# naturerobots/mesh_navigation

Measured on NVIDIA H100. Metric: vertex-relaxations/sec, higher is better.
Workload: dtype f64 update / f32 store

## Files before the change

mesh_navigation_b200/csrc/band_engine.cuh:

```cuda
#pragma once
#include <cooperative_groups.h>
#include <cstdint>

#include "wavefront_math.cuh"

namespace mnb {
namespace cg = cooperative_groups;

constexpr uint32_t INF_BITS = 0x7f800000u;
constexpr int STAGNATION_ROUNDS = 24;

constexpr uint32_t EXT_POOL = 0x80000000u;
struct EvTime { float a1, a2, a3; uint32_t root, ext, self; };
__device__ __forceinline__ EvTime ev_normal(float key, uint32_t id) { EvTime t; t.a1 = key; t.a2 = 0.0f; t.a3 = 0.0f; t.root = id; t.ext = 0u; t.self = id; return t; }
struct Label { float d; EvTime t; };
__device__ __forceinline__ uint4 state_inf() { return make_uint4(INF_BITS, INF_BITS, 0u, 0u); }

struct TimeAlg {
  const uint32_t* pool = nullptr;
  __device__ __forceinline__ uint32_t id2_of(const EvTime& t) const {
    return t.a3 == 0.0f ? t.self : ((t.ext & EXT_POOL) ? __ldcg(&pool[(t.ext & ~EXT_POOL) + 1]) : t.ext);
  }
  __device__ __forceinline__ uint32_t id3_of(const EvTime& t) const {
    return (t.ext & EXT_POOL) ? __ldcg(&pool[(t.ext & ~EXT_POOL) + 2]) : t.self;
  }
  __device__ __forceinline__ uint32_t levels_of(const EvTime& t) const {
    return t.a2 == 0.0f ? 1u : (t.a3 == 0.0f ? 2u : ((t.ext & EXT_POOL) ? __ldcg(&pool[t.ext & ~EXT_POOL]) : 3u));
  }
  __device__ __noinline__ bool less_tail(const EvTime x, const EvTime y) const {
    const uint32_t i2x = id2_of(x), i2y = id2_of(y);
    if (i2x != i2y) return i2x < i2y;
    if (x.a3 != y.a3) return x.a3 < y.a3;
    if (x.a3 == 0.0f) return false;
    const uint32_t i3x = id3_of(x), i3y = id3_of(y);
    if (i3x != i3y) return i3x < i3y;
    const uint32_t nx = levels_of(x), ny = levels_of(y);
    const uint32_t ox = x.ext & ~EXT_POOL, oy = y.ext & ~EXT_POOL;
    for (uint32_t i = 4;; ++i) {
      if (i > nx) return i <= ny;
      if (i > ny) return false;
      const uint32_t kx = __ldcg(&pool[ox + 3 + 2 * (i - 4)]), ky = __ldcg(&pool[oy + 3 + 2 * (i - 4)]);
      if (kx != ky) return kx < ky;
      const uint32_t ix = __ldcg(&pool[ox + 4 + 2 * (i - 4)]), iy = __ldcg(&pool[oy + 4 + 2 * (i - 4)]);
      if (ix != iy) return ix < iy;
    }
// ... 180 lines not shown
};

template <int CS>
__device__ __forceinline__ void group_sync(unsigned int* bar = nullptr) {
  if constexpr (CS == 1) {
    __syncthreads();
  } else if constexpr (CS == 0) {
    (void)bar;
    cg::this_grid().sync();
  } else {
    cg::this_cluster().sync();
  }
}

template <int CAP_>
struct StageT {
  static constexpr int CAP = CAP_;
  static constexpr int SW_CAP = 1024;
  uint32_t buf[CAP];
  unsigned int n;
  unsigned int base;
  unsigned int m_tau;
  unsigned int lo;
};
using Stage = StageT<3072>;
struct SweepStage {
  uint32_t seen[Stage::SW_CAP];
  uint4 lab[Stage::SW_CAP];
  uint16_t dl[Stage::SW_CAP];
  unsigned int dn[2];
};
constexpr uint32_t SEEN_NEVER = 0xffffffffu;

__device__ __forceinline__ unsigned int stage_push(Stage& st, uint32_t v, uint32_t* list_next, unsigned int* count_next) {
  const unsigned int p = atomicAdd(&st.n, 1u);
  if (p < Stage::CAP) st.buf[p] = v;
  else list_next[atomicAdd(count_next, 1u)] = v;
  return p;
}
__device__ __forceinline__ void stage_push_seen(Stage& st, SweepStage& ss, uint32_t v, uint32_t seen, const uint4& label_bits,
                                                uint32_t* list_next, unsigned int* count_next) {
  const unsigned int p = stage_push(st, v, list_next, count_next);
  if (p < Stage::SW_CAP) { ss.seen[p] = seen; ss.lab[p] = label_bits; }
}

template <class S>
__device__ __forceinline__ void stage_flush(S& st, uint32_t* list_next, unsigned int* count_next,
                                            unsigned int* g_m_tau, unsigned int* g_lo) {
  __syncthreads();
  const unsigned int n = st.n < (unsigned)S::CAP ? st.n : (unsigned)S::CAP;
  if (threadIdx.x == 0) {
    st.base = n ? atomicAdd(count_next, n) : 0u;
    if (st.m_tau != INF_BITS) atomicMin(g_m_tau, st.m_tau);
    if (st.lo != INF_BITS) atomicMin(g_lo, st.lo);
  }
  __syncthreads();
  const unsigned int base = st.base;
  for (unsigned int i = threadIdx.x; i < n; i += blockDim.x) list_next[base + i] = st.buf[i];
  __syncthreads();
  if (threadIdx.x == 0) { st.n = 0; st.m_tau = INF_BITS; st.lo = INF_BITS; }
}

template <int CS, class P>
__device__ void run_band_rounds(P& prob, GroupCtl* ctl, uint32_t* list0, uint32_t* list1, uint32_t* mark,
                                Stage& st, const float delta, const uint32_t gthreads, const uint32_t gtid,
                                const int has_robot, const uint32_t r0, const uint32_t r1, const uint32_t r2,
                                const double goal_dist_offset, const volatile int* cancel_flag,
                                const float band_end_init, const uint32_t max_rounds) {
  float band_end_prev = band_end_init;
  unsigned long long my_recomputes = 0, my_settled = 0, my_skipped = 0;
  float lo_best = -1.0f; int stagnant = 0;
  prob.strict = 0;
  uint32_t r = 0;
  for (;; ++r) {
    const uint32_t slot = r % 3, prev = (r + 2) % 3, next = (r + 1) % 3;
    const unsigned int n = __ldcg(&ctl->count[slot]);
// ... 124 lines not shown
    {
      my_mtau = fminf(my_mtau, prob.deferred_m);
      prob.deferred_m = __uint_as_float(INF_BITS);
      const unsigned int wm = __reduce_min_sync(0xffffffffu, __float_as_uint(my_mtau));
      const unsigned int wl = __reduce_min_sync(0xffffffffu, __float_as_uint(my_lo));
      if ((threadIdx.x & 31) == 0) {
        if (wm != INF_BITS) atomicMin(&st.m_tau, wm);
        if (wl != INF_BITS) atomicMin(&st.lo, wl);
      }
    }
    stage_flush(st, list_n, &ctl->count[next], &ctl->m_tau[slot], &ctl->lo[slot]);
    band_end_prev = band_end;
    group_sync<CS>(ctl->barrier);
  }
  atomicAdd(&ctl->recomputes, my_recomputes);
  atomicAdd(&ctl->settled, my_settled);
  if (my_skipped) atomicAdd(&ctl->skipped, my_skipped);
  if (gtid == 0) {
    ctl->rounds += r;
    if (prob.strict) ctl->strict_armed += 1;
    if (r > max_rounds) ctl->watchdog = 1;
    ctl->goal_bits = min(ctl->goal_ring[0], ctl->goal_ring[1]);
  }
}

template <int CS, bool SW, class P>
__device__ void run_band_rounds_sub8(P& prob, GroupCtl* ctl, uint32_t* list0, uint32_t* list1, uint32_t* mark,
                                     Stage& st, const float delta, const uint32_t gthreads, const uint32_t gtid,
                                     const int has_robot, const uint32_t r0, const uint32_t r1, const uint32_t r2,
                                     const double goal_dist_offset, const volatile int* cancel_flag,
                                     const float band_end_init, const uint32_t max_rounds, const int n_sweeps_arg,
                                     SweepStage* ss, const uint32_t n_vertices) {
  const int n_sweeps = SW ? n_sweeps_arg : 0;
  bool rescanned = false;
  float band_end_prev = band_end_init;
  unsigned long long my_recomputes = 0, my_settled = 0, my_skipped = 0;
  float lo_best = -1.0f; int stagnant = 0;
  prob.strict = 0;
  const uint32_t j = threadIdx.x & 7;
  const uint32_t nblk = gthreads / blockDim.x, blk = gtid / blockDim.x;
  uint32_t r = 0;
  for (;; ++r) {
    const uint32_t slot = r % 3, prev = (r + 2) % 3, next = (r + 1) % 3;
    const unsigned int n = __ldcg(&ctl->count[slot]);
    const float m_prev = __uint_as_float(__ldcg(&ctl->m_tau[prev]));
    const float lo_prev = __uint_as_float(__ldcg(&ctl->lo[prev]));
    const unsigned int goal_b = __ldcg(&ctl->goal_ring[r & 1]);
    const float goal = __uint_as_float(goal_b);
    if constexpr (P::HAS_GOAL_TIME) if (has_robot && goal_b != INF_BITS) {
      prob.goal_t.a1 = __uint_as_float(__ldcg(&ctl->goal_time[0])); prob.goal_t.root = __ldcg(&ctl->goal_time[1]);
      prob.goal_t.a2 = __uint_as_float(__ldcg(&ctl->goal_time[2])); prob.goal_t.a3 = __uint_as_float(__ldcg(&ctl->goal_time[3]));
      prob.goal_t.ext = __ldcg(&ctl->goal_time[4]); prob.goal_t.self = __ldcg(&ctl->goal_time[5]);
    }
    const unsigned int stop = __ldcg(&ctl->stop_ring[r & 1]);
    const bool need_rescan = has_robot && goal_b != INF_BITS && !rescanned;
    if (stop || r > max_rounds) break;
    if (!need_rescan && n == 0) break;
    if (!need_rescan && r > 0 && __float_as_uint(m_prev) == INF_BITS &&
        (__float_as_uint(lo_prev) == INF_BITS || lo_prev > goal)) break;
    if (r > 0 && __float_as_uint(m_prev) != INF_BITS && !(lo_prev > lo_best)) { if (++stagnant >= STAGNATION_ROUNDS) prob.strict = 1; }
    else { stagnant = 0; if (lo_prev > lo_best) lo_best = lo_prev; }
#ifdef MNB_EMU_ACTIVE
    if (gtid == 0 && getenv("MNB_EMU_TRACE")) fprintf(stderr, "[round %u] list %u m_prev %g lo_prev %g strict %d\n", r, n, m_prev, lo_prev, prob.strict);
#endif
    float delta_r = delta;
    if constexpr (SW) {
// ... 56 lines not shown
          my_mtau = fminf(my_mtau, fminf(tau, nt.a1));
        }
        my_lo = fminf(my_lo, nt.a1);
        if constexpr (SW) {
          if (fresh) stage_push_seen(st, *ss, c, v0, prob.pack_label(c, nd, nt), list_n, &ctl->count[next]);
          else if (changed) ss->lab[slot] = prob.pack_label(c, nd, nt);
        } else {
          stage_push(st, c, list_n, &ctl->count[next]);
        }
      }
      if constexpr (SW) if (n_sweeps > 0) {
        __syncwarp();
        if (changed) {
          if (ix.x != -1 && deg <= 8) { atomicAdd(&prob.ver[ix.x], 1u); if constexpr (P::TWO_SOURCES) atomicAdd(&prob.ver[ix.y], 1u); }
          if (j == 0 && deg > 8) prob.activate(c, [&](uint32_t x) { atomicAdd(&prob.ver[x], 1u); });
        }
      }
      if (has && __float_as_uint(nd) != INF_BITS && mk == MARK_CAND) {
        if (ix.x != -1) {
          if (!prob.prefetch_marks) { mk1 = __ldcg(&mark[ix.x]); if (P::TWO_SOURCES) mk2 = __ldcg(&mark[ix.y]); }
          if (mk1 == MARK_NONE && prob.eligible((uint32_t)ix.x) && atomicCAS(&mark[ix.x], MARK_NONE, MARK_CAND) == MARK_NONE)
            { if constexpr (SW) stage_push_seen(st, *ss, (uint32_t)ix.x, SEEN_NEVER, state_inf(), list_n, &ctl->count[next]); else stage_push(st, (uint32_t)ix.x, list_n, &ctl->count[next]); }
          if (P::TWO_SOURCES && mk2 == MARK_NONE && prob.eligible((uint32_t)ix.y) && atomicCAS(&mark[ix.y], MARK_NONE, MARK_CAND) == MARK_NONE)
            { if constexpr (SW) stage_push_seen(st, *ss, (uint32_t)ix.y, SEEN_NEVER, state_inf(), list_n, &ctl->count[next]); else stage_push(st, (uint32_t)ix.y, list_n, &ctl->count[next]); }
        }
        if (j == 0 && deg > 8)
          prob.activate(c, [&](uint32_t x) {
            if (__ldcg(&mark[x]) == MARK_NONE && prob.eligible(x) && atomicCAS(&mark[x], MARK_NONE, MARK_CAND) == MARK_NONE)
              { if constexpr (SW) stage_push_seen(st, *ss, x, SEEN_NEVER, state_inf(), list_n, &ctl->count[next]); else stage_push(st, x, list_n, &ctl->count[next]); }
          });
        if (j == 0) mark[c] = MARK_CAND_ACT;
      }
    };
    const unsigned int cnt = n > blk ? (n - blk + nblk - 1) / nblk : 0u;
    for (unsigned int qb = (threadIdx.x >> 5) * 4u; qb < cnt; qb += (blockDim.x >> 3)) {
      const unsigned int q = qb + ((threadIdx.x & 31) >> 3);
      bool has = q < cnt;
      uint32_t c = 0;
      if (has) c = __ldcg(&list_r[(size_t)q * nblk + blk]);
      Label old = prob.load_label(has ? c : 0u);
      int4 ix = prob.load_row_idx(has ? c : 0u, j);
      float4 w = prob.load_row_w(has ? c : 0u, j);
      const uint32_t mk = __ldcg(&mark[has ? c : 0u]);
      uint32_t v0 = 0;
      if constexpr (SW) if (n_sweeps > 0) v0 = __ldcg(&prob.ver[has ? c : 0u]);
      const float d = old.d, tau = old.t.a1;
      if (has && tau < m_prev && tau < band_end_prev && tau < settle_cap) {
        if (j == 0) {
          mark[c] = MARK_FIXED;
          my_settled++;
          if (has_robot && (c == r0 || c == r1 || c == r2)) {
            if (atomicSub(&ctl->robot_left, 1) == 1) {
              float bd = d; EvTime bt = old.t;
              const uint32_t rv[3] = {r0, r1, r2};
              for (int k = 0; k < 3; ++k) {
                const Label so = prob.load_label(rv[k]);
                if (prob.tless(bt, so.t)) { bt = so.t; bd = so.d; }
              }
              ctl->goal_time[0] = __float_as_uint(bt.a1); ctl->goal_time[1] = bt.root; ctl->goal_time[2] = __float_as_uint(bt.a2);
            ctl->goal_time[3] = __float_as_uint(bt.a3); ctl->goal_time[4] = bt.ext; ctl->goal_time[5] = bt.self;
            atomicMin(&ctl->goal_ring[(r + 1) & 1], __float_as_uint((float)((double)bd + goal_dist_offset)));
            }
          }
        }
        has = false;
      }
      if constexpr (P::CAN_SKIP) if (skip_ok && has) {
        const uint32_t le = __ldcg(&prob.last_eval[c]), dr = __ldcg(&prob.dirty_round[c]);
        const float em = __uint_as_float(__ldcg(&prob.excl_min[c]));
        if (le != 0u && dr < le && !(band_end > em)) {
          if (j == 0) {
            my_lo = fminf(my_lo, tau);
            my_skipped++;
            if constexpr (SW) stage_push_seen(st, *ss, c, v0, prob.pack_label(c, old.d, old.t), list_n, &ctl->count[next]);
            else stage_push(st, c, list_n, &ctl->count[next]);
          }
          has = false;
        }
      }
      evaluate(has, c, old, ix, w, mk, v0, true, 0u);
    }
#ifdef MNB_GRID_TIMING
    const long long tps = clock64();
#endif
#ifdef MNB_GRID_TIMING
    if (gtid == 0) { ctl->t_ph[0] += (unsigned long long)(tps - tp0); ctl->t_ph[2] += cnt; }
#endif
    if constexpr (SW) for (int sw = 0; sw < n_sweeps; ++sw) {
#ifdef MNB_GRID_TIMING
      const long long tq0 = clock64();
#endif
      __syncthreads();
      const unsigned int ns = min(st.n, (unsigned int)Stage::SW_CAP);
      unsigned int* dcur = &ss->dn[sw & 1];
      if (threadIdx.x == 0) ss->dn[(sw + 1) & 1] = 0;
      for (unsigned int i = threadIdx.x; i < ns; i += blockDim.x) {
        const uint32_t c = st.buf[i];
        const uint32_t v0 = __ldcg(&prob.ver[c]);
        if (v0 != ss->seen[i]) { ss->seen[i] = v0; ss->dl[atomicAdd(dcur, 1u)] = (uint16_t)i; }
      }
      __syncthreads();
      const unsigned int dn = *dcur;
#ifdef MNB_GRID_TIMING
      const long long tq1 = clock64();
#endif
#ifdef MNB_GRID_TIMING
      if (gtid == 0) { ctl->t_ph[3] += dn; ctl->t_ph[4] += ns; ctl->t_ph[5] += (unsigned long long)(tq1 - tq0); }
#endif
      for (unsigned int ib = (threadIdx.x >> 5) * 4u; ib < dn; ib += (blockDim.x >> 3)) {
        const unsigned int i = ib + ((threadIdx.x & 31) >> 3);
        const bool has = i < dn;
        const uint32_t slot = has ? ss->dl[i] : 0u;
        const uint32_t c = has ? st.buf[slot] : 0u;
        const Label old = has ? prob.unpack_label(c, ss->lab[slot]) : prob.unpack_label(0u, state_inf());
// ... 46 lines not shown
```

mesh_navigation_b200/csrc/batch_engine.cuh:

```cuda
#pragma once
#include "problems.cuh"

namespace mnb {

struct BatchSeeds { uint32_t s0, s1, s2, noexpand; float seed_max; };
constexpr uint32_t LIST_ACTIVATED = 0x80000000u;

struct BatchGroup {
  uint4* state; uint32_t* root_arr; uint32_t* ext_arr; uint32_t* chg; uint32_t* mark; uint32_t* pool; uint32_t pool_cap; GroupCtl* ctl;
  uint4* skipw;
};

template <class Args>
__device__ __forceinline__ void batch_make_problem(const Args& a, const BatchGroup& G, const BatchSeeds& sd, int strict,
                                                   CvpEllProblemT<false>& prob) {
  prob.cor_ptr = a.cor_ptr; prob.cor_idx = a.cor_idx; prob.cor_w = a.cor_w; prob.cost = a.cost; prob.invalid = a.invalid;
  prob.ell_idx = a.ell_idx; prob.ell_w = a.ell_w; prob.ell_geo = a.ell_geo;
  prob.state = G.state; prob.ext_arr = G.ext_arr; prob.root_arr = G.root_arr; prob.chg = G.chg;
  prob.pool_w = G.pool; prob.pool = G.pool; prob.pool_cap = G.pool_cap; prob.pool_top = &G.ctl->pool_top; prob.pool_overflow = &G.ctl->pool_overflow;
  prob.ver = nullptr; prob.deferred_m = __uint_as_float(INF_BITS); prob.pred = nullptr; prob.dir = nullptr; prob.cut = nullptr;
  prob.cost_limit = a.cost_limit; prob.s0 = sd.s0; prob.s1 = sd.s1; prob.s2 = sd.s2; prob.seed_noexpand = sd.noexpand; prob.seed_max_d = sd.seed_max;
  prob.goal_t = ev_normal(__uint_as_float(INF_BITS), 0u);
  prob.last_eval = nullptr; prob.dirty_round = nullptr; prob.excl_min = nullptr; prob.skip_clean = 0; prob.prefetch_marks = false;
  prob.strict = strict;
// ... 246 lines not shown
          tau = __uint_as_float(__ldcg(reinterpret_cast<const uint32_t*>(G.state) + 4 * (size_t)c + 1));
          settled = tau < m_prev && tau < band_end_prev;
          if (!settled) {
            const uint4 sk = __ldcg(&G.skipw[c]);
            const uint32_t dmb = buf_prev ? sk.y : sk.x;
            if (dmb != INF_BITS) __stcg(&skw[4 * (size_t)c + buf_prev], INF_BITS);
            clean = !strict && !(__uint_as_float(dmb) <= tau) && !(band_end > __uint_as_float(sk.z));
          }
        }
        if (settled) my_settled++;
        const bool keep = has && !settled && clean, work = has && !settled && !clean;
        if (keep) { my_skipped++; my_lo = fminf(my_lo, tau); }
        const unsigned km = __ballot_sync(FULL, keep), wm = __ballot_sync(FULL, work);
        if (km) {
          unsigned int base = 0;
          if (lane == 0) base = atomicAdd(&st.n, (unsigned)__popc(km));
          base = __shfl_sync(FULL, base, 0);
          if (keep) batch_stage_write(st, base + __popc(km & lt), ce, list_n, count_next);
        }
        if (wm) {
          unsigned int base = 0;
          if (lane == 0) base = atomicAdd(&wk.n, (unsigned)__popc(wm));
          base = __shfl_sync(FULL, base, 0);
          if (work) wk.q[base + __popc(wm & lt)] = ce;
        }
      }
      __syncthreads();
      const unsigned int nwork = wk.n;
      for (unsigned int ib = (threadIdx.x & ~31u); ib < nwork; ib += blockDim.x) {
        const unsigned int i = ib + lane;
        const bool has = i < nwork;
        bool defer = false;
        uint32_t ce = 0u, c = 0u; uint4 ob = make_uint4(0u, 0u, 0u, 0u);
        float m = INF, tmin_nc = INF, excl = INF; int deg = 0;
        if (has) {
          ce = wk.q[i]; c = ce & ~LIST_ACTIVATED;
          ob = __ldcg(&G.state[c]);
          if (strict) defer = true;
          for (int k = 0; k < (int)ELL_W && !defer; ++k) {
            const int4 ix = __ldg(&a.ell_idx[(size_t)c * ELL_W + k]);
            if (k == 0) { deg = ix.w; if (deg > (int)ELL_W) { defer = true; break; } }
            if (ix.x == ELL_EMPTY) continue;
            const uint32_t v1 = (uint32_t)ix.x, v2 = (uint32_t)ix.y;
            const uint4 sa = __ldcg(&G.state[v1]), sb = __ldcg(&G.state[v2]);
            const float da = __uint_as_float(sa.x), db = __uint_as_float(sb.x);
            if (((sa.z | sa.w | sb.z | sb.w) >> 31) || da <= sd.seed_max || db <= sd.seed_max) { defer = true; break; }
            if (a.invalid && (a.invalid[v1] || a.invalid[v2])) continue;
            if (sa.x != INF_BITS && !(da < band_end)) excl = fminf(excl, da);
            if (sb.x != INF_BITS && !(db < band_end)) excl = fminf(excl, db);
            if (!(da < band_end) || !(db < band_end)) continue;
            const float ta = __uint_as_float(sa.y), tb = __uint_as_float(sb.y);
            const bool v1_later = tb < ta || (tb == ta && v2 < v1);
            const float T1 = v1_later ? ta : tb;
            const float4 w = __ldg(&a.ell_w[(size_t)c * ELL_W + k]);
            double U, X;
#ifdef MNB_BATCH_GEO_TABLE
            const double2* gp = reinterpret_cast<const double2*>(a.ell_geo) + 2 * ((size_t)c * ELL_W + k);
            const double2 g01 = __ldg(gp), g23 = __ldg(gp + 1);
            CvpEllProblemT<false>::FaceGeo fg; fg.p = g01.x; fg.hc = g01.y; fg.t0a = g23.x;
            CvpEllProblemT<false>::eval_face_geo((double)da, (double)db, (double)w.z, (double)w.y, (double)w.x, fg, U, X);
#else
            CvpEllProblemT<false>::eval_face((double)da, (double)db, (double)w.z, (double)w.y, (double)w.x, U, X);
#endif
            const float Xf = (float)X;
            if (Xf > T1 && U <= X) m = fminf(m, Xf); else tmin_nc = fminf(tmin_nc, T1);
          }
          if (!defer && __float_as_uint(tmin_nc) != INF_BITS && !(tmin_nc > m)) defer = true;
        }
        const bool done = has && !defer;
        bool changed = false, act_now = false;
        if (done) {
          const float tau = __uint_as_float(ob.y);
          const uint32_t mb = __float_as_uint(m);
          changed = ob.x != mb || ob.y != mb || ob.z != 0u || ob.w != 0u;
          if (changed) {
            if (ob.x != INF_BITS) __stcg(&G.chg[c], r + 1u);
            __stcg(&G.state[c], make_uint4(mb, mb, 0u, 0u));
            my_mtau = fminf(my_mtau, fminf(tau, m));
          }
          __stcg(&skw[4 * (size_t)c + 2], __float_as_uint(excl <= m ? excl : INF));
          my_recomputes++;
          my_lo = fminf(my_lo, m);
          act_now = !(ce & LIST_ACTIVATED) && mb != INF_BITS;
          if (changed || act_now) {
            const uint32_t kb = __float_as_uint(fminf(tau, m));
#ifndef MNB_BATCH_SERIAL_ACTIVATION
            uint32_t todo = 0u;
            if (act_now) {
#pragma unroll
              for (int k = 0; k < (int)ELL_W; ++k) {
                const int4 ix = __ldg(&a.ell_idx[(size_t)c * ELL_W + k]);
                if (ix.x == ELL_EMPTY) continue;
                if (__ldcg(&G.mark[(uint32_t)ix.x]) == MARK_NONE) todo |= 1u << (2 * k);
                if (__ldcg(&G.mark[(uint32_t)ix.y]) == MARK_NONE) todo |= 2u << (2 * k);
              }
            }
            for (int k = 0; k < (int)ELL_W; ++k) {
              const int4 ix = __ldg(&a.ell_idx[(size_t)c * ELL_W + k]);
              if (ix.x == ELL_EMPTY) continue;
              const uint32_t xs[2] = {(uint32_t)ix.x, (uint32_t)ix.y};
// ... 80 lines not shown
```

mesh_navigation_b200/csrc/meshnav.cu:

```cuda
#include <cuda_runtime.h>

#include <algorithm>
#include <functional>
#include <cmath>
#include <cstdio>
#include <cstring>
#include <string>
#include <vector>

#include "../../include/meshnav_b200.h"
#include "band_engine.cuh"
#include "problems.cuh"
#include "topology.hpp"

using namespace mnb;

#include "launch.cuh"
#include "kernels_maps.cuh"
#include "kernels_wavefront.cuh"
#include "kernels_layers.cuh"
#include "kernels_field.cuh"
#include "kernels_updates.cuh"
#include "kernels_raycast.cuh"

// ... 453 lines not shown
  (void)stream;
  return emu::launch(kern, blocks, (unsigned)threads, (size_t)0, 1u, true, args);
#else
  void* kargs[] = {(void*)&args};
  return cudaLaunchCooperativeKernel((const void*)kern, dim3(blocks), dim3(threads), kargs, 0, stream);
#endif
}

static int32_t launch_cvp(mnb_ctx* ctx, const CvpKernelArgs& a, int cs, unsigned groups) {
  cudaError_t e;
  const unsigned blocks = groups * cs;
  const int threads = MNB_CVP_THREADS;
  switch (cs) {
    case 1: e = launch_cluster(k_cvp<1, false>, a, 1, blocks, threads, ctx->stream); break;
    case 2: e = launch_cluster(k_cvp<2, false>, a, 2, blocks, threads, ctx->stream); break;
    case 4: e = launch_cluster(k_cvp<4, false>, a, 4, blocks, threads, ctx->stream); break;
    case 8: e = launch_cluster(k_cvp<8, false>, a, 8, blocks, threads, ctx->stream); break;
    default: e = launch_cluster(k_cvp<16, false>, a, 16, blocks, threads, ctx->stream); break;
  }
  if (e != cudaSuccess) { ctx->err = std::string("cvp launch: ") + cudaGetErrorString(e); return MNB_E_CUDA; }
  return MNB_OK;
}

static int32_t finish_stats(mnb_ctx* ctx, unsigned groups, unsigned launches) {
  std::vector<GroupCtl> h(groups);
  CK(cudaMemcpyAsync(h.data(), ctx->ws.ctl, sizeof(GroupCtl) * groups, cudaMemcpyDeviceToHost, ctx->stream));
  CK(cudaStreamSynchronize(ctx->stream));
  ctx->stats.rounds = 0; ctx->stats.recomputes = 0; ctx->stats.settled = 0;
  ctx->stats.skipped = 0; ctx->stats.deep_labels = 0; ctx->stats.pool_words = 0;
  for (auto& c : h) { ctx->stats.deep_labels += c.deep_labels; ctx->stats.pool_words = std::max<uint64_t>(ctx->stats.pool_words, c.pool_top); }
  for (auto& c : h) { ctx->stats.rounds += c.rounds; ctx->stats.recomputes += c.recomputes; ctx->stats.settled += c.settled; ctx->stats.skipped += c.skipped; }
  ctx->stats.kernel_launches = launches;
  float ms = 0; cudaEventElapsedTime(&ms, ctx->ev0, ctx->ev1); ctx->stats.kernel_ms = ms;
  if (getenv("MNB_PHASE_TIMING")) for (auto& c : h) fprintf(stderr, "[mnb] rounds %llu: CTA0 cycles work %llu flush %llu sync %llu (per round %.0f / %.0f / %.0f) main-pass cycles %llu (unused %llu) chunk-candidates %llu | sweeps: dirty %llu polled %llu poll-cycles %llu eval-cycles %llu (%llu)\n", c.rounds, c.t_work, c.t_flush, c.t_sync, (double)c.t_work / (double)(c.rounds ? c.rounds : 1), (double)c.t_flush / (double)(c.rounds ? c.rounds : 1), (double)c.t_sync / (double)(c.rounds ? c.rounds : 1), c.t_ph[0], c.t_ph[1], c.t_ph[2], c.t_ph[3], c.t_ph[4], c.t_ph[5], c.t_ph[6], c.t_ph[7]);
  for (auto& c : h)
    if (c.watchdog) { ctx->err = "wavefront did not converge within the round watchdog"; return MNB_E_STATE; }
  for (auto& c : h)
    if (c.pool_overflow) { ctx->err = "level pool exhausted: the cascades of this map nest deeper than the workspace holds (result discarded)"; return MNB_E_NOMEM; }
  return MNB_OK;
}

static int32_t ensure_out(mnb_ctx* ctx, size_t n_dist, bool aux) {
  if (n_dist > ctx->out_dist_cap) { dfree(ctx->d_out_dist); CK(dalloc(&ctx->d_out_dist, n_dist)); ctx->out_dist_cap = n_dist; }
  if (aux && !ctx->d_out_pred) {
    CK(dalloc(&ctx->d_out_pred, (size_t)ctx->V)); CK(dalloc(&ctx->d_out_dir, (size_t)ctx->V)); CK(dalloc(&ctx->d_out_cut, (size_t)ctx->V));
  }
  return MNB_OK;
}

static int32_t ensure_seeds(mnb_ctx* ctx, uint32_t n) {
  if (n > ctx->seed_cap) {
    dfree(ctx->d_seed_faces); dfree(ctx->d_seed_pos);
    CK(dalloc(&ctx->d_seed_faces, (size_t)n)); CK(dalloc(&ctx->d_seed_pos, 3 * (size_t)n));
    ctx->seed_cap = n;
  }
  return MNB_OK;
}

static void fill_cvp_args(mnb_ctx* ctx, CvpKernelArgs& a) {
  a.V = ctx->V; a.pos = ctx->d_pos; a.faces = ctx->d_faces; a.cor_ptr = ctx->d_cor_ptr; a.cor_idx = ctx->d_cor_idx;
  a.cor_w = ctx->d_cor_w; a.ell_idx = ctx->d_ell_idx; a.ell_w = ctx->d_ell_w; a.ell_geo = ctx->d_ell_geo; a.cost = ctx->d_cost; a.invalid = ctx->has_invalid ? ctx->d_invalid : nullptr; a.ws = ctx->ws;
  a.seed_faces = ctx->d_seed_faces; a.seed_pos = ctx->d_seed_pos; a.delta = ctx->delta; a.next_query = ctx->d_next_query;
  a.cancel_flag = ctx->d_cancel; a.max_rounds = watchdog_rounds(ctx->V); a.sweeps = 0; a.skip_clean = ctx->skip_clean;
  a.hop = ctx->w_mean > 0 ? 1.35f * ctx->w_mean : 0.16f;
}

extern "C" {
// ... 690 lines not shown
```

mesh_navigation_b200/csrc/problems.cuh:

```cuda
#pragma once
#include "band_engine.cuh"

namespace mnb {

struct CvpProblem : LabelStore {
  static constexpr bool CAN_SKIP = false;
  static constexpr bool HAS_GOAL_TIME = true;
  EvTime goal_t;
  static constexpr int STAGNATION = STAGNATION_ROUNDS;
  const uint32_t* __restrict__ cor_ptr;
  const int4* __restrict__ cor_idx;
  const float4* __restrict__ cor_w;
  const float* __restrict__ cost;
  const uint8_t* __restrict__ invalid;
  uint32_t* pred;
  float* dir;
  int32_t* cut;
  double cost_limit;
  uint32_t s0, s1, s2;
  uint32_t seed_noexpand;
  float seed_max_d = __builtin_huge_valf();

  static constexpr int MAXF = 12;

// ... 110 lines not shown
    int n = 0;
    for (uint32_t k = kb; k < ke; ++k) {
      EvTime T; float u1, u2; uint32_t Tv;
      if (!corner_time(c, k, band_end, goal, T, Tv, u1, u2)) continue;
      Tt[n] = T; U1[n] = u1; U2[n] = u2; K[n] = k; TV[n] = Tv; ++n;
    }
    float cur = __uint_as_float(INF_BITS);
    EvFull tc = full_normal(cur, c);
    for (int i = 0; i < n; ++i) {
      int b = i;
      for (int j = i + 1; j < n; ++j)
        if (tless(Tt[j], Tt[b]) || (teq(Tt[j], Tt[b]) && K[j] < K[b])) b = j;
      const EvTime T = Tt[b]; const float u1 = U1[b], u2 = U2[b]; const uint32_t k = K[b], Tv = TV[b];
      Tt[b] = Tt[i]; U1[b] = U1[i]; U2[b] = U2[i]; K[b] = K[i]; TV[b] = TV[i];
      if (!less_T_full(T, tc)) break;
      const float4 w = __ldg(&cor_w[k]);
      CvpResult r;
      if (cvp_update_t<false>(u1, u2, cur, w.z, w.y, w.x, r) && backstep_ok(r.value, T, Tv, round)) { cur = r.value; accept(c, r.value, T, tc); win = (int)k; wu1 = u1; wu2 = u2; }
    }
    nd = cur; nt = tc;
  }

  __device__ __forceinline__ bool recompute(uint32_t c, float band_end, float goal, uint32_t round, const Label& old, float& nd, float& ntau) {
    int win; float wu1, wu2; EvFull nf;
    replay(c, band_end, goal, round, nd, nf, win, wu1, wu2);
    const EvTime nt = finish(nf, old.t);
    ntau = nt.a1;
    if (__float_as_uint(nd) == __float_as_uint(old.d) && teq(nt, old.t)) return false;
    store_label(c, nd, nt, __float_as_uint(old.d) != INF_BITS, round);
    return true;
  }
};

constexpr uint32_t ELL_W = 8;
constexpr int ELL_EMPTY = -1;

template <bool SKIP>
struct CvpEllProblemT : CvpProblem {
  static constexpr bool TWO_SOURCES = true;
  static constexpr bool CAN_SKIP = SKIP;
  uint32_t* last_eval;
  uint32_t* dirty_round;
  uint32_t* excl_min;
  int skip_clean;
  bool prefetch_marks;
  const int4* __restrict__ ell_idx;
  const float4* __restrict__ ell_w;
  const double4* __restrict__ ell_geo;

  __device__ __forceinline__ static void eval_face(double u1, double u2, double a, double b, double c, double& U, double& X) {
    const double c_sq = c * c, b_sq = b * b, a_sq = a * a;
    const double u1_sq = u1 * u1, u2_sq = u2 * u2;
    const double sx = (c_sq + u1_sq - u2_sq) / (2 * c);
    const double sy = -sqrt(fmax(u1_sq - sx * sx, 0.0));
    const double p = (b_sq + c_sq - a_sq) / (2 * c);
    const double hc = sqrt(fmax(b_sq - p * p, 0.0));
    const double dy = hc - sy;
    const double dx = p - sx;
    const double u3tmp_sq = dx * dx + dy * dy;
    const double u3tmp = sqrt(u3tmp_sq);
    U = u3tmp;
    const double t0a = (a_sq + b_sq - c_sq) / (2 * a * b);
    const double t1a = (u3tmp_sq + b_sq - u1_sq) / (2 * u3tmp * b);
    const double t2a = (a_sq + u3tmp_sq - u2_sq) / (2 * a * u3tmp);
    int fb;
    if (fabs(t1a) > 1) fb = 1;
    else if (fabs(t2a) > 1) fb = 2;
    else if (fabs(t0a) <= 1 && acos_less(t1a, t0a) && acos_less(t2a, t0a)) { X = u3tmp; return; }
    else fb = acos_less(t1a, t2a) ? 1 : 2;
    X = (fb == 1) ? (u1 + b) : (u2 + a);
  }

  template <class F>
  __device__ __forceinline__ void activate_lane(uint32_t c, uint32_t j, const int4& ix, int deg, F push) const {
    if (ix.x != ELL_EMPTY) { push((uint32_t)ix.x); push((uint32_t)ix.y); }
    if (j == 0 && deg > (int)ELL_W) activate(c, push);
  }

  __device__ __noinline__ void replay_serial(uint32_t c, float band_end, float goal, uint32_t round, const EvTime& old_t, float& nd, EvTime& nt) const {
    int win; float a1, a2; EvFull nf;
    replay(c, band_end, goal, round, nd, nf, win, a1, a2);
    nt = finish(nf, old_t);
  }

  __device__ __forceinline__ int4 load_row_idx(uint32_t c, uint32_t j) const { return __ldg(&ell_idx[(size_t)c * ELL_W + j]); }
  __device__ __forceinline__ float4 load_row_w(uint32_t c, uint32_t j) const { return __ldg(&ell_w[(size_t)c * ELL_W + j]); }

  struct FaceGeo { double p, hc, t0a; };
  __device__ __forceinline__ static FaceGeo face_geo(double a, double b, double c) {
    const double c_sq = c * c, b_sq = b * b, a_sq = a * a;
    FaceGeo g;
    g.p = (b_sq + c_sq - a_sq) / (2 * c);
    g.hc = sqrt(fmax(b_sq - g.p * g.p, 0.0));
    g.t0a = (a_sq + b_sq - c_sq) / (2 * a * b);
    return g;
  }
  __device__ __forceinline__ static void eval_face_geo(double u1, double u2, double a, double b, double c, const FaceGeo& g,
                                                       double& U, double& X) {
    const double c_sq = c * c, b_sq = b * b, a_sq = a * a;
    const double u1_sq = u1 * u1, u2_sq = u2 * u2;
    const double sx = (c_sq + u1_sq - u2_sq) / (2 * c);
    const double sy = -sqrt(fmax(u1_sq - sx * sx, 0.0));
    const double dy = g.hc - sy;
// ... 352 lines not shown
  }

  __device__ __forceinline__ bool recompute(uint32_t c, float band_end, float goal, uint32_t , const Label& old, float& nd, float& ntau) {
    const uint32_t kb = adj_ptr[c], ke = adj_ptr[c + 1];
    float best = __uint_as_float(INF_BITS), best_du = best; uint32_t best_u = c;
    for (uint32_t k = kb; k < ke; ++k) {
      const uint2 nw = __ldg(&adj_nw[k]);
      const uint32_t u = nw.x;
      const float du = __uint_as_float(__ldcg(&state[u]).x);
      if (!(du < band_end)) continue;
      if (du > goal) continue;
      if ((double)__ldg(&cost[u]) > cost_limit) continue;
      const float tmp = __fadd_rn(du, __uint_as_float(nw.y));
      if (tmp < best || (tmp == best && __float_as_uint(tmp) != INF_BITS &&
                         (du < best_du || (du == best_du && u < best_u)))) {
        best = tmp; best_du = du; best_u = u;
      }
    }
    nd = best; ntau = best;
    if (__float_as_uint(nd) == __float_as_uint(old.d)) {
      if (__float_as_uint(nd) != INF_BITS && pred[c] != best_u) pred[c] = best_u;
      return false;
    }
    __stcg(&state[c], make_uint4(__float_as_uint(nd), __float_as_uint(ntau), 0u, 0u));
    pred[c] = best_u;
    return true;
  }
};


struct DijkstraEllProblem : DijkstraProblem {
  static constexpr bool TWO_SOURCES = false;
  static constexpr bool CAN_SKIP = false;
  uint32_t* last_eval = nullptr; uint32_t* dirty_round = nullptr; uint32_t* excl_min = nullptr; int skip_clean = 0;
  static constexpr bool prefetch_marks = true;
  const uint4* __restrict__ ell_adj;
  uint32_t* ver;

  __device__ __forceinline__ int4 load_row_idx(uint32_t c, uint32_t j) const {
    const uint4 r = __ldg(&ell_adj[(size_t)c * ELL_W + j]);
    return make_int4((int)r.x, (int)r.y, 0, (int)r.w);
  }
  __device__ __forceinline__ float4 load_row_w(uint32_t, uint32_t) const { return make_float4(0.f, 0.f, 0.f, 0.f); }
  __device__ __forceinline__ uint4 pack_label(uint32_t, float d, const EvTime& t) const {
    return make_uint4(__float_as_uint(d), __float_as_uint(t.a1), 0u, 0u);
  }
  __device__ __forceinline__ Label unpack_label(uint32_t v, const uint4& s) const {
    Label l; l.d = __uint_as_float(s.x); l.t = ev_normal(__uint_as_float(s.y), v);
    return l;
  }
  __device__ __forceinline__ void store_label(uint32_t c, float d, const EvTime& t, bool, uint32_t) const {
    __stcg(&state[c], make_uint4(__float_as_uint(d), __float_as_uint(t.a1), 0u, 0u));
  }
  __device__ __forceinline__ static bool better(float tmp, float du, uint32_t u, float best, float best_du, uint32_t best_u) {
    return tmp < best || (tmp == best && __float_as_uint(tmp) != INF_BITS && (du < best_du || (du == best_du && u < best_u)));
  }
  __device__ __noinline__ void replay_serial(uint32_t c, float band_end, float goal, float& best, uint32_t& best_u) const {
    const uint32_t kb = adj_ptr[c], ke = adj_ptr[c + 1];
    best = __uint_as_float(INF_BITS); float best_du = best; best_u = c;
    for (uint32_t k = kb; k < ke; ++k) {
      const uint2 nw = __ldg(&adj_nw[k]);
      const uint32_t u = nw.x;
      const float du = __uint_as_float(__ldcg(&state[u]).x);
      if (!(du < band_end) || du > goal || (double)__ldg(&cost[u]) > cost_limit) continue;
      const float tmp = __fadd_rn(du, __uint_as_float(nw.y));
      if (better(tmp, du, u, best, best_du, best_u)) { best = tmp; best_du = du; best_u = u; }
// ... 37 lines not shown
```

Measured before the change: 124.0 million.

## Add one-thread-per-vertex fast path for plain faces in banded sweep rounds

In sweep rounds for the non-skip CVP problem, each warp first handles vertices one per thread using a shared plain-face evaluator. Relaxation, activation of neighbours and staging use a warp prefix sum with one shared atomic per warp. Vertices that cannot be resolved on this path (high degree, non-plain state, non-convex faces, strict or goal rounds) are queued in shared memory and reprocessed by the existing 8-lanes-per-vertex pass. This targets the lane underuse of the 8-wide pass on typical low-degree vertices, at the cost of extra shared memory, block syncs per chunk and divergence inside the per-thread face loop. The batch engine is refactored to reuse the same evaluator.

```diff
diff --git a/mesh_navigation_b200/csrc/band_engine.cuh b/mesh_navigation_b200/csrc/band_engine.cuh
--- a/mesh_navigation_b200/csrc/band_engine.cuh
+++ b/mesh_navigation_b200/csrc/band_engine.cuh
@@ -11,6 +11,8 @@
 constexpr int STAGNATION_ROUNDS = 24;
 
 constexpr uint32_t EXT_POOL = 0x80000000u;
+constexpr uint32_t ELL_W = 8;
+constexpr int ELL_EMPTY = -1;
 struct EvTime { float a1, a2, a3; uint32_t root, ext, self; };
 __device__ __forceinline__ EvTime ev_normal(float key, uint32_t id) { EvTime t; t.a1 = key; t.a2 = 0.0f; t.a3 = 0.0f; t.root = id; t.ext = 0u; t.self = id; return t; }
 struct Label { float d; EvTime t; };
@@ -257,16 +259,23 @@
 };
 constexpr uint32_t SEEN_NEVER = 0xffffffffu;
 
+__device__ __forceinline__ void stage_put(Stage& st, unsigned int p, uint32_t v, uint32_t* list_next, unsigned int* count_next) {
+  if (p < Stage::CAP) st.buf[p] = v;
+  else list_next[atomicAdd(count_next, 1u)] = v;
+}
 __device__ __forceinline__ unsigned int stage_push(Stage& st, uint32_t v, uint32_t* list_next, unsigned int* count_next) {
   const unsigned int p = atomicAdd(&st.n, 1u);
-  if (p < Stage::CAP) st.buf[p] = v;
-  else list_next[atomicAdd(count_next, 1u)] = v;
+  stage_put(st, p, v, list_next, count_next);
   return p;
+}
+__device__ __forceinline__ void stage_put_seen(Stage& st, SweepStage& ss, unsigned int p, uint32_t v, uint32_t seen, const uint4& label_bits,
+                                               uint32_t* list_next, unsigned int* count_next) {
+  stage_put(st, p, v, list_next, count_next);
+  if (p < Stage::SW_CAP) { ss.seen[p] = seen; ss.lab[p] = label_bits; }
 }
 __device__ __forceinline__ void stage_push_seen(Stage& st, SweepStage& ss, uint32_t v, uint32_t seen, const uint4& label_bits,
                                                 uint32_t* list_next, unsigned int* count_next) {
-  const unsigned int p = stage_push(st, v, list_next, count_next);
-  if (p < Stage::SW_CAP) { ss.seen[p] = seen; ss.lab[p] = label_bits; }
+  stage_put_seen(st, ss, atomicAdd(&st.n, 1u), v, seen, label_bits, list_next, count_next);
 }
 
 template <class S>
@@ -457,6 +466,10 @@
                                      const float band_end_init, const uint32_t max_rounds, const int n_sweeps_arg,
                                      SweepStage* ss, const uint32_t n_vertices) {
   const int n_sweeps = SW ? n_sweeps_arg : 0;
+  constexpr bool FAST = SW && P::PLAIN_FAST;
+  __shared__ uint32_t gq[FAST ? Stage::SW_CAP : 1];
+  __shared__ unsigned int gq_n;
+  if constexpr (FAST) { if (threadIdx.x == 0) gq_n = 0; __syncthreads(); }
   bool rescanned = false;
   float band_end_prev = band_end_init;
   unsigned long long my_recomputes = 0, my_settled = 0, my_skipped = 0;
@@ -579,37 +592,39 @@
         if (j == 0) mark[c] = MARK_CAND_ACT;
       }
     };
+    auto settle = [&](const uint32_t c, const Label& old) {
+      mark[c] = MARK_FIXED;
+      my_settled++;
+      if (has_robot && (c == r0 || c == r1 || c == r2)) {
+        if (atomicSub(&ctl->robot_left, 1) == 1) {
+          float bd = old.d; EvTime bt = old.t;
+          const uint32_t rv[3] = {r0, r1, r2};
+          for (int k = 0; k < 3; ++k) {
+            const Label so = prob.load_label(rv[k]);
+            if (prob.tless(bt, so.t)) { bt = so.t; bd = so.d; }
+          }
+          ctl->goal_time[0] = __float_as_uint(bt.a1); ctl->goal_time[1] = bt.root; ctl->goal_time[2] = __float_as_uint(bt.a2);
+          ctl->goal_time[3] = __float_as_uint(bt.a3); ctl->goal_time[4] = bt.ext; ctl->goal_time[5] = bt.self;
+          atomicMin(&ctl->goal_ring[(r + 1) & 1], __float_as_uint((float)((double)bd + goal_dist_offset)));
+        }
+      }
+    };
     const unsigned int cnt = n > blk ? (n - blk + nblk - 1) / nblk : 0u;
-    for (unsigned int qb = (threadIdx.x >> 5) * 4u; qb < cnt; qb += (blockDim.x >> 3)) {
+    auto main_pass8 = [&](const unsigned int cnt_g, const bool queued) {
+    for (unsigned int qb = (threadIdx.x >> 5) * 4u; qb < cnt_g; qb += (blockDim.x >> 3)) {
       const unsigned int q = qb + ((threadIdx.x & 31) >> 3);
-      bool has = q < cnt;
+      bool has = q < cnt_g;
       uint32_t c = 0;
-      if (has) c = __ldcg(&list_r[(size_t)q * nblk + blk]);
+      if (has) c = queued ? gq[q] : __ldcg(&list_r[(size_t)q * nblk + blk]);
       Label old = prob.load_label(has ? c : 0u);
       int4 ix = prob.load_row_idx(has ? c : 0u, j);
       float4 w = prob.load_row_w(has ? c : 0u, j);
       const uint32_t mk = __ldcg(&mark[has ? c : 0u]);
       uint32_t v0 = 0;
       if constexpr (SW) if (n_sweeps > 0) v0 = __ldcg(&prob.ver[has ? c : 0u]);
-      const float d = old.d, tau = old.t.a1;
+      const float tau = old.t.a1;
       if (has && tau < m_prev && tau < band_end_prev && tau < settle_cap) {
-        if (j == 0) {
-          mark[c] = MARK_FIXED;
-          my_settled++;
-          if (has_robot && (c == r0 || c == r1 || c == r2)) {
-            if (atomicSub(&ctl->robot_left, 1) == 1) {
-              float bd = d; EvTime bt = old.t;
-              const uint32_t rv[3] = {r0, r1, r2};
-              for (int k = 0; k < 3; ++k) {
-                const Label so = prob.load_label(rv[k]);
-                if (prob.tless(bt, so.t)) { bt = so.t; bd = so.d; }
-              }
-              ctl->goal_time[0] = __float_as_uint(bt.a1); ctl->goal_time[1] = bt.root; ctl->goal_time[2] = __float_as_uint(bt.a2);
-            ctl->goal_time[3] = __float_as_uint(bt.a3); ctl->goal_time[4] = bt.ext; ctl->goal_time[5] = bt.self;
-            atomicMin(&ctl->goal_ring[(r + 1) & 1], __float_as_uint((float)((double)bd + goal_dist_offset)));
-            }
-          }
-        }
+        if (j == 0) settle(c, old);
         has = false;
       }
       if constexpr (P::CAN_SKIP) if (skip_ok && has) {
@@ -627,6 +642,108 @@
       }
       evaluate(has, c, old, ix, w, mk, v0, true, 0u);
     }
+    };
+    if constexpr (FAST) {
+      constexpr unsigned FULL = 0xffffffffu;
+      const uint32_t lane = threadIdx.x & 31u, lt = (1u << lane) - 1u;
+      const bool fast_round = !prob.strict && !(has_robot && goal_b != INF_BITS);
+      for (unsigned int cb = 0; cb < cnt; cb += (unsigned)Stage::SW_CAP) {
+        const unsigned int ce = min(cnt, cb + (unsigned)Stage::SW_CAP);
+        for (unsigned int ib = cb + (threadIdx.x & ~31u); ib < ce; ib += blockDim.x) {
+          const unsigned int i = ib + lane;
+          bool has = i < ce;
+          uint32_t c = 0u, mk = MARK_FIXED, v0 = 0u;
+          uint4 ob = make_uint4(0u, 0u, 0u, 0u);
+          if (has) {
+            c = __ldcg(&list_r[(size_t)i * nblk + blk]);
+            ob = __ldcg(&prob.state[c]);
+            mk = __ldcg(&mark[c]);
+            if (n_sweeps > 0) v0 = __ldcg(&prob.ver[c]);
+            const float tau = __uint_as_float(ob.y);
+            if (tau < m_prev && tau < band_end_prev && tau < settle_cap) { settle(c, prob.unpack_label(c, ob)); has = false; }
+          }
+          float m = 0.0f, excl;
+          const bool done = has && fast_round &&
+              P::eval_plain(prob.ell_idx, prob.ell_w, prob.ell_geo, prob.invalid, prob.state, prob.seed_max_d, band_end, c, m, excl);
+          const uint32_t mb = __float_as_uint(m);
+          const uint4 nb = make_uint4(mb, mb, 0u, 0u);
+          uint32_t won = 0u;
+          if (done) {
+            const bool changed = ob.x != mb || ob.y != mb || ob.z != 0u || ob.w != 0u;
+            my_recomputes++;
+            if (changed) {
+              if (ob.x != INF_BITS) __stcg(&prob.chg[c], r + 1u);
+              __stcg(&prob.state[c], nb);
+              my_mtau = fminf(my_mtau, fminf(__uint_as_float(ob.y), m));
+            }
+            my_lo = fminf(my_lo, m);
+            const bool act = mb != INF_BITS && mk == MARK_CAND;
+            const bool bump = changed && n_sweeps > 0;
+            if (bump || act) {
+              uint32_t todo = 0u;
+              if (act) {
+#pragma unroll
+                for (int k = 0; k < (int)ELL_W; ++k) {
+                  const int4 ix = prob.load_row_idx(c, (uint32_t)k);
+                  if (ix.x == ELL_EMPTY) continue;
+                  if (__ldcg(&mark[(uint32_t)ix.x]) == MARK_NONE) todo |= 1u << (2 * k);
+                  if (__ldcg(&mark[(uint32_t)ix.y]) == MARK_NONE) todo |= 2u << (2 * k);
+                }
+              }
+#pragma unroll
+              for (int k = 0; k < (int)ELL_W; ++k) {
+                const int4 ix = prob.load_row_idx(c, (uint32_t)k);
+                if (ix.x == ELL_EMPTY) continue;
+                const uint32_t xs[2] = {(uint32_t)ix.x, (uint32_t)ix.y};
+#pragma unroll
+                for (int t = 0; t < 2; ++t) {
+                  const uint32_t x = xs[t];
+                  if (bump) atomicAdd(&prob.ver[x], 1u);
+                  if (((todo >> (2 * k + t)) & 1u) && prob.eligible(x) && atomicCAS(&mark[x], MARK_NONE, MARK_CAND) == MARK_NONE)
+                    won |= 1u << (2 * k + t);
+                }
+              }
+              if (act) mark[c] = MARK_CAND_ACT;
+            }
+          }
+          const unsigned int mine = (done ? 1u : 0u) + (unsigned)__popc(won);
+          unsigned int incl = mine;
+#pragma unroll
+          for (int o = 1; o < 32; o <<= 1) { const unsigned int y = __shfl_up_sync(FULL, incl, o); if (lane >= (unsigned)o) incl += y; }
+          const unsigned int tot = __shfl_sync(FULL, incl, 31);
+          if (tot) {
+            unsigned int base = 0u;
+            if (lane == 0) base = atomicAdd(&st.n, tot);
+            unsigned int p = __shfl_sync(FULL, base, 0) + incl - mine;
+            if (done) stage_put_seen(st, *ss, p++, c, v0, nb, list_n, &ctl->count[next]);
+            for (; won; won &= won - 1u) {
+              const int b = __ffs(won) - 1;
+              const int4 ix = prob.load_row_idx(c, (uint32_t)(b >> 1));
+              stage_put_seen(st, *ss, p++, (b & 1) ? (uint32_t)ix.y : (uint32_t)ix.x, SEEN_NEVER, state_inf(), list_n, &ctl->count[next]);
+            }
+          }
+          const bool defer = has && !done;
+          const unsigned dq = __ballot_sync(FULL, defer);
+          if (dq) {
+            unsigned int qbase = 0u;
+            if (lane == 0) qbase = atomicAdd(&gq_n, (unsigned)__popc(dq));
+            qbase = __shfl_sync(FULL, qbase, 0);
+            if (defer) gq[qbase + __popc(dq & lt)] = c;
+          }
+        }
+        __syncthreads();
+        const unsigned int nq = gq_n;
+#ifdef MNB_GRID_TIMING
+        if (gtid == 0) { ctl->t_ph[1] += nq; ctl->t_ph[7] += (unsigned long long)(clock64() - tp0); }
+#endif
+        main_pass8(nq, true);
+        __syncthreads();
+        if (threadIdx.x == 0) gq_n = 0;
+        __syncthreads();
+      }
+    } else {
+      main_pass8(cnt, false);
+    }
 #ifdef MNB_GRID_TIMING
     const long long tps = clock64();
 #endif
diff --git a/mesh_navigation_b200/csrc/batch_engine.cuh b/mesh_navigation_b200/csrc/batch_engine.cuh
--- a/mesh_navigation_b200/csrc/batch_engine.cuh
+++ b/mesh_navigation_b200/csrc/batch_engine.cuh
@@ -302,40 +302,11 @@
         const bool has = i < nwork;
         bool defer = false;
         uint32_t ce = 0u, c = 0u; uint4 ob = make_uint4(0u, 0u, 0u, 0u);
-        float m = INF, tmin_nc = INF, excl = INF; int deg = 0;
+        float m = INF, excl = INF;
         if (has) {
           ce = wk.q[i]; c = ce & ~LIST_ACTIVATED;
           ob = __ldcg(&G.state[c]);
-          if (strict) defer = true;
-          for (int k = 0; k < (int)ELL_W && !defer; ++k) {
-            const int4 ix = __ldg(&a.ell_idx[(size_t)c * ELL_W + k]);
-            if (k == 0) { deg = ix.w; if (deg > (int)ELL_W) { defer = true; break; } }
-            if (ix.x == ELL_EMPTY) continue;
-            const uint32_t v1 = (uint32_t)ix.x, v2 = (uint32_t)ix.y;
-            const uint4 sa = __ldcg(&G.state[v1]), sb = __ldcg(&G.state[v2]);
-            const float da = __uint_as_float(sa.x), db = __uint_as_float(sb.x);
-            if (((sa.z | sa.w | sb.z | sb.w) >> 31) || da <= sd.seed_max || db <= sd.seed_max) { defer = true; break; }
-            if (a.invalid && (a.invalid[v1] || a.invalid[v2])) continue;
-            if (sa.x != INF_BITS && !(da < band_end)) excl = fminf(excl, da);
-            if (sb.x != INF_BITS && !(db < band_end)) excl = fminf(excl, db);
-            if (!(da < band_end) || !(db < band_end)) continue;
-            const float ta = __uint_as_float(sa.y), tb = __uint_as_float(sb.y);
-            const bool v1_later = tb < ta || (tb == ta && v2 < v1);
-            const float T1 = v1_later ? ta : tb;
-            const float4 w = __ldg(&a.ell_w[(size_t)c * ELL_W + k]);
-            double U, X;
-#ifdef MNB_BATCH_GEO_TABLE
-            const double2* gp = reinterpret_cast<const double2*>(a.ell_geo) + 2 * ((size_t)c * ELL_W + k);
-            const double2 g01 = __ldg(gp), g23 = __ldg(gp + 1);
-            CvpEllProblemT<false>::FaceGeo fg; fg.p = g01.x; fg.hc = g01.y; fg.t0a = g23.x;
-            CvpEllProblemT<false>::eval_face_geo((double)da, (double)db, (double)w.z, (double)w.y, (double)w.x, fg, U, X);
-#else
-            CvpEllProblemT<false>::eval_face((double)da, (double)db, (double)w.z, (double)w.y, (double)w.x, U, X);
-#endif
-            const float Xf = (float)X;
-            if (Xf > T1 && U <= X) m = fminf(m, Xf); else tmin_nc = fminf(tmin_nc, T1);
-          }
-          if (!defer && __float_as_uint(tmin_nc) != INF_BITS && !(tmin_nc > m)) defer = true;
+          defer = strict || !CvpEllProblemT<false>::eval_plain(a.ell_idx, a.ell_w, a.ell_geo, a.invalid, G.state, sd.seed_max, band_end, c, m, excl);
         }
         const bool done = has && !defer;
         bool changed = false, act_now = false;
diff --git a/mesh_navigation_b200/csrc/meshnav.cu b/mesh_navigation_b200/csrc/meshnav.cu
--- a/mesh_navigation_b200/csrc/meshnav.cu
+++ b/mesh_navigation_b200/csrc/meshnav.cu
@@ -509,7 +509,7 @@
   for (auto& c : h) { ctx->stats.rounds += c.rounds; ctx->stats.recomputes += c.recomputes; ctx->stats.settled += c.settled; ctx->stats.skipped += c.skipped; }
   ctx->stats.kernel_launches = launches;
   float ms = 0; cudaEventElapsedTime(&ms, ctx->ev0, ctx->ev1); ctx->stats.kernel_ms = ms;
-  if (getenv("MNB_PHASE_TIMING")) for (auto& c : h) fprintf(stderr, "[mnb] rounds %llu: CTA0 cycles work %llu flush %llu sync %llu (per round %.0f / %.0f / %.0f) main-pass cycles %llu (unused %llu) chunk-candidates %llu | sweeps: dirty %llu polled %llu poll-cycles %llu eval-cycles %llu (%llu)\n", c.rounds, c.t_work, c.t_flush, c.t_sync, (double)c.t_work / (double)(c.rounds ? c.rounds : 1), (double)c.t_flush / (double)(c.rounds ? c.rounds : 1), (double)c.t_sync / (double)(c.rounds ? c.rounds : 1), c.t_ph[0], c.t_ph[1], c.t_ph[2], c.t_ph[3], c.t_ph[4], c.t_ph[5], c.t_ph[6], c.t_ph[7]);
+  if (getenv("MNB_PHASE_TIMING")) for (auto& c : h) fprintf(stderr, "[mnb] rounds %llu: CTA0 cycles work %llu flush %llu sync %llu (per round %.0f / %.0f / %.0f) main-pass cycles %llu candidates %llu (queued for 8 lanes %llu) | sweeps: dirty %llu polled %llu poll-cycles %llu eval-cycles %llu | main pass, one-thread phase cycles %llu\n", c.rounds, c.t_work, c.t_flush, c.t_sync, (double)c.t_work / (double)(c.rounds ? c.rounds : 1), (double)c.t_flush / (double)(c.rounds ? c.rounds : 1), (double)c.t_sync / (double)(c.rounds ? c.rounds : 1), c.t_ph[0], c.t_ph[2], c.t_ph[1], c.t_ph[3], c.t_ph[4], c.t_ph[5], c.t_ph[6], c.t_ph[7]);
   for (auto& c : h)
     if (c.watchdog) { ctx->err = "wavefront did not converge within the round watchdog"; return MNB_E_STATE; }
   for (auto& c : h)
diff --git a/mesh_navigation_b200/csrc/problems.cuh b/mesh_navigation_b200/csrc/problems.cuh
--- a/mesh_navigation_b200/csrc/problems.cuh
+++ b/mesh_navigation_b200/csrc/problems.cuh
@@ -166,13 +166,12 @@
   }
 };
 
-constexpr uint32_t ELL_W = 8;
-constexpr int ELL_EMPTY = -1;
 
 template <bool SKIP>
 struct CvpEllProblemT : CvpProblem {
   static constexpr bool TWO_SOURCES = true;
   static constexpr bool CAN_SKIP = SKIP;
+  static constexpr bool PLAIN_FAST = !SKIP;
   uint32_t* last_eval;
   uint32_t* dirty_round;
   uint32_t* excl_min;
@@ -203,6 +202,45 @@
     else if (fabs(t0a) <= 1 && acos_less(t1a, t0a) && acos_less(t2a, t0a)) { X = u3tmp; return; }
     else fb = acos_less(t1a, t2a) ? 1 : 2;
     X = (fb == 1) ? (u1 + b) : (u2 + a);
+  }
+
+  __device__ __forceinline__ static bool eval_plain(const int4* __restrict__ ell_idx, const float4* __restrict__ ell_w,
+                                                    const double4* __restrict__ ell_geo, const uint8_t* __restrict__ invalid,
+                                                    const uint4* state, float seed_max, float band_end, uint32_t c,
+                                                    float& m, float& excl) {
+    (void)ell_geo;
+    const float INF = __uint_as_float(INF_BITS);
+    float tmin_nc = INF;
+    m = INF; excl = INF;
+    for (int k = 0; k < (int)ELL_W; ++k) {
+      const int4 ix = __ldg(&ell_idx[(size_t)c * ELL_W + k]);
+      if (k == 0 && ix.w > (int)ELL_W) return false;
+      if (ix.x == ELL_EMPTY) continue;
+      const uint32_t v1 = (uint32_t)ix.x, v2 = (uint32_t)ix.y;
+      const uint4 sa = __ldcg(&state[v1]), sb = __ldcg(&state[v2]);
+      const float da = __uint_as_float(sa.x), db = __uint_as_float(sb.x);
+      if (((sa.z | sa.w | sb.z | sb.w) >> 31) || da <= seed_max || db <= seed_max) return false;
+      if (invalid && (invalid[v1] || invalid[v2])) continue;
+      if (sa.x != INF_BITS && !(da < band_end)) excl = fminf(excl, da);
+      if (sb.x != INF_BITS && !(db < band_end)) excl = fminf(excl, db);
+      if (!(da < band_end) || !(db < band_end)) continue;
+      const float ta = __uint_as_float(sa.y), tb = __uint_as_float(sb.y);
+      const bool v1_later = tb < ta || (tb == ta && v2 < v1);
+      const float T1 = v1_later ? ta : tb;
+      const float4 w = __ldg(&ell_w[(size_t)c * ELL_W + k]);
+      double U, X;
+#ifdef MNB_BATCH_GEO_TABLE
+      const double2* gp = reinterpret_cast<const double2*>(ell_geo) + 2 * ((size_t)c * ELL_W + k);
+      const double2 g01 = __ldg(gp), g23 = __ldg(gp + 1);
+      FaceGeo fg; fg.p = g01.x; fg.hc = g01.y; fg.t0a = g23.x;
+      eval_face_geo((double)da, (double)db, (double)w.z, (double)w.y, (double)w.x, fg, U, X);
+#else
+      eval_face((double)da, (double)db, (double)w.z, (double)w.y, (double)w.x, U, X);
+#endif
+      const float Xf = (float)X;
+      if (Xf > T1 && U <= X) m = fminf(m, Xf); else tmin_nc = fminf(tmin_nc, T1);
+    }
+    return __float_as_uint(tmin_nc) == INF_BITS || tmin_nc > m;
   }
 
   template <class F>
@@ -621,6 +659,7 @@
 struct DijkstraEllProblem : DijkstraProblem {
   static constexpr bool TWO_SOURCES = false;
   static constexpr bool CAN_SKIP = false;
+  static constexpr bool PLAIN_FAST = false;
   uint32_t* last_eval = nullptr; uint32_t* dirty_round = nullptr; uint32_t* excl_min = nullptr; int skip_clean = 0;
   static constexpr bool prefetch_marks = true;
   const uint4* __restrict__ ell_adj;
```

Measured after the change: 128.7 million, median of 6. 1.04x the previous value.
